# salesforce/ALPRO

Hardware: AMD Instinct MI355X
Metric: video-text pairs/sec (8f x 224^2, 40-tok) (higher is better)
Workload: dtype fp16

## Files before the change

alpro_amd/csrc/attention.hip:

```cpp
#include "common.hpp"
#include "attn_tile.hpp"

namespace alpro {
namespace {

template <typename T> __device__ __forceinline__ int k_swz(int row, int chunk) {
  if (TileCfg<T>::CPR == 8) return chunk ^ ((row >> 1) & 7);
  return chunk ^ (row & 15);
}

template <typename T> struct Col4;
template <> struct Col4<float> {
  typedef u32x4 type;
  static __device__ __forceinline__ u32x4 load(const char* v, int key0, int d) {
    const float* p = (const float*)(v + key0 * TileCfg<float>::RB) + d;
    return mk4(f2u(p[0]), f2u(p[64]), f2u(p[128]), f2u(p[192]));
  }
};
template <typename T16> struct Col4_16 {
  typedef u32x2 type;
  static __device__ __forceinline__ u32x2 load(const char* v, int key0, int d) {
    const uint16_t* p = (const uint16_t*)(v + key0 * (HD * 2)) + d;
    u32x2 r;
    r.x = (uint32_t)p[0] | ((uint32_t)p[64] << 16);
// ... 156 lines not shown
      for (int r = 0; r < 16; ++r) s[kt][r] = 0.f;
      const int krow = kt * 32 + ql;
#pragma unroll
      for (int ks = 0; ks < C::KS; ++ks) {
        const u32x4 a = *(const u32x4*)(Ks + krow * C::RB + (k_swz<T>(krow, 2 * ks + g) << 4));
        mma_chunk<T>(s[kt], a, qf[ks]);
      }
      __builtin_amdgcn_sched_barrier(0);
    }
    const float l_se = softmax_tiles<NKT>(s, scale, [&](int kt, int rq) { return *(const float4*)(Bs + kt * 32 + 8 * rq + 4 * g); });
    if (lse && g == 0 && q < L) lse[((int64_t)b * H + h) * L + q] = l_se;
    if (drop_seed) {
      const uint32_t th = drop_thresh24(drop_p);
      const float ks = 1.0f / (1.0f - drop_p);
      const uint64_t base_i = (((uint64_t)b * H + h) * L + (uint64_t)qc) * L;
#pragma unroll
      for (int kt = 0; kt < NKT; ++kt)
#pragma unroll
        for (int r = 0; r < 16; ++r) s[kt][r] = drop_keep(drop_seed, base_i + kt * 32 + acc_row(r, lane), th) ? s[kt][r] * ks : 0.f;
    }

    f32x16 o[2];
#pragma unroll
    for (int dt = 0; dt < 2; ++dt)
#pragma unroll
      for (int r = 0; r < 16; ++r) o[dt][r] = 0.f;
    pv_tiles<T, NKT>(o, s, Vs, lane);
    if (q < L) store_row64<T>(out + ((int64_t)b * L + q) * H * HD + h * HD, o, lane);
  }
}

__device__ u32x4 g_attn_zero[4];

template <typename T> struct ClsSplit;
template <> struct ClsSplit<f16_t> { static constexpr int NS = 2; static constexpr float C1 = 2048.f, C2 = 1.f; };
template <> struct ClsSplit<bf16_t> { static constexpr int NS = 3; static constexpr float C1 = 1.f, C2 = 1.f; };
template <typename T> __device__ __forceinline__ void cls_split(float x, float& p0, float& p1, float& p2) {
  p0 = quantize<T>(x);
  const float r1 = (x - p0) * ClsSplit<T>::C1;
  p1 = quantize<T>(r1);
  p2 = ClsSplit<T>::NS == 3 ? quantize<T>((r1 - p1) * ClsSplit<T>::C2) : 0.f;
}
template <typename T> struct ClsTrunc;
template <> struct ClsTrunc<f16_t> { static constexpr uint32_t MASK = 0xFFFFE000u; };
template <> struct ClsTrunc<bf16_t> { static constexpr uint32_t MASK = 0xFFFF0000u; };
__device__ __forceinline__ float and_bits(float x, uint32_t m) { return __builtin_bit_cast(float, __builtin_bit_cast(uint32_t, x) & m); }

template <typename T> __device__ __forceinline__ float cls_join(float v0, float v1, float v2) {
  float r = fmaf(v1, 1.0f / ClsSplit<T>::C1, v0);
  if (ClsSplit<T>::NS == 3) r = fmaf(v2, 1.0f / (ClsSplit<T>::C1 * ClsSplit<T>::C2), r);
  return r;
}

template <int N> __device__ __forceinline__ float dpp_from_above(float v) {
  return __builtin_bit_cast(float, __builtin_amdgcn_update_dpp(0, __builtin_bit_cast(int, v), 0x100 + N, 0xf, 0xf, true));
}
template <int N> __device__ __forceinline__ float dpp_from_below(float v) {
  return __builtin_bit_cast(float, __builtin_amdgcn_update_dpp(0, __builtin_bit_cast(int, v), 0x110 + N, 0xf, 0xf, true));
}

template <typename T, int NKT, bool HAS_BIAS, bool CLS = false, bool DROP = false>
__global__ __launch_bounds__(256, 2) void attn_fwd16_kernel(const T* __restrict__ qkv, T* __restrict__ out, int L, int H, float scale,
                                                            const float* __restrict__ key_bias, float* __restrict__ lse, float drop_p,
                                                            uint32_t drop_seed, int order, const float* __restrict__ cls_q, int cls_group,
                                                            float* __restrict__ cls_out) {
  static_assert(sizeof(T) == 2, "16-bit storage only");
  constexpr int LP = NKT * 32, RB = 128;
  constexpr int NS = ClsSplit<T>::NS;
  extern __shared__ __attribute__((aligned(16))) char smem[];
  char* Ks = smem;
  char* Vs = smem + LP * RB;
  char* Os = smem + 2 * LP * RB;
  constexpr bool HALF = NKT == 8;
  constexpr int OW = HALF ? 2048 : 4096;
  float* Bs = (float*)(Os + 4 * OW);
  const int tid = threadIdx.x, lane = tid & 63, wave = __builtin_amdgcn_readfirstlane(tid >> 6);
  int b, h;
  attn_unit(blockIdx.x, gridDim.x, H, order, b, h);
  for (int c = tid; c < LP; c += 256) Bs[c] = c < L ? (HAS_BIAS ? key_bias[(int64_t)b * L + c] * LOG2E : 0.f) : -INFINITY;
  const int64_t ldq = 3 * (int64_t)H * HD;
  const T* base = qkv + (int64_t)b * L * ldq + h * HD;
  const int nqt = (L + 31) >> 5;
  const int g = lane >> 5, ql = lane & 31;

  int cls_tile = -1, c0 = 0, ntile = nqt;
  if (CLS && cls_q) {
    c0 = L - 32 * (nqt - 1);
    if ((c0 & 15) + NS > 16) c0 = (c0 | 15) + 1;
    cls_tile = nqt - 1;
    if (c0 + NS > 32) { c0 = 0; cls_tile = nqt; ntile = nqt + 1; }
  }

// ... 364 lines not shown
                  const float* cls_q, int cls_group, float* cls_out, hipStream_t st) {
  const int nkt = (L + 31) / 32;
  if constexpr (sizeof(T) == 2) {
#define ALPRO_ATTN16(N)                                                                                       \
  return key_bias ? launch_attn16<T, N, true>(qkv, out, batch, L, H, scale, key_bias, lse, dp, ds, cls_q, cls_group, cls_out, st)         \
                  : launch_attn16<T, N, false>(qkv, out, batch, L, H, scale, key_bias, lse, dp, ds, cls_q, cls_group, cls_out, st)
    if (nkt <= 2) ALPRO_ATTN16(2);
    if (nkt <= 4) ALPRO_ATTN16(4);
    if (nkt <= 7) ALPRO_ATTN16(7);
    ALPRO_ATTN16(8);
#undef ALPRO_ATTN16
  }
  if (nkt <= 2) return launch_attn<T, 2>(qkv, out, batch, L, H, scale, key_bias, lse, dp, ds, st);
  if (nkt <= 4) return launch_attn<T, 4>(qkv, out, batch, L, H, scale, key_bias, lse, dp, ds, st);
  if (nkt <= 7) return launch_attn<T, 7>(qkv, out, batch, L, H, scale, key_bias, lse, dp, ds, st);
  return launch_attn<T, 8>(qkv, out, batch, L, H, scale, key_bias, lse, dp, ds, st);
}

}
}

using namespace alpro;

extern "C" int alpro_attn_fwd(const void* qkv, void* out, int dtype, int batch, int L, int H, float scale,
                              const float* key_bias, float* lse, float drop_p, uint32_t drop_seed, const float* cls_q, int cls_group, float* cls_out,
                              void* stream) {
  ALPRO_CHECK(!cls_q || (cls_out && cls_group > 0 && batch % cls_group == 0 && dtype != ALPRO_F32 && ((uintptr_t)cls_q % 16) == 0 && ((uintptr_t)cls_out % 16) == 0),
              "alpro_attn_fwd: the precise CLS query needs cls_out, a group size dividing the batch, 16-byte aligned fp32 side tensors and a 16-bit operand dtype");
  ALPRO_CHECK(qkv && out && batch > 0 && H > 0, "alpro_attn_fwd: bad args");
  ALPRO_CHECK(L > 0 && L <= ALPRO_ATTN_MAX_L, "alpro_attn_fwd: L=%d unsupported (1..%d = ALPRO_ATTN_MAX_L)", L, ALPRO_ATTN_MAX_L);
  ALPRO_CHECK(((uintptr_t)qkv % 16) == 0 && ((uintptr_t)out % 16) == 0, "alpro_attn_fwd: pointers must be 16-byte aligned");
  ALPRO_CHECK(!drop_seed || (drop_p > 0.f && drop_p < 1.f), "alpro_attn_fwd: dropout needs 0 < p < 1");
  if (L > 256) return attn_long_fwd(qkv, out, dtype, batch, L, H, scale, key_bias, lse, drop_p, drop_seed, cls_q, cls_group, cls_out, (hipStream_t)stream);
  ALPRO_DISPATCH_DTYPE(dtype, T, return dispatch_attn<T>(qkv, out, batch, L, H, scale, key_bias, lse, drop_p, drop_seed, cls_q, cls_group, cls_out, (hipStream_t)stream));
  return ALPRO_OK;
}

extern "C" int alpro_attn_temporal_fwd_drop(const void* qkv, void* out, int dtype, int64_t rows, int T, int H, float scale, float* lse, float drop_p,
                                            uint32_t drop_seed, void* stream) {
  ALPRO_CHECK(qkv && out && rows > 0 && H > 0, "alpro_attn_temporal_fwd: bad args");
  ALPRO_CHECK(T > 0 && T <= ALPRO_ATTN_MAX_T, "alpro_attn_temporal_fwd: num_frm=%d unsupported (1..%d = ALPRO_ATTN_MAX_T)", T, ALPRO_ATTN_MAX_T);
  ALPRO_CHECK(rows % T == 0, "alpro_attn_temporal_fwd: rows=%lld not a multiple of T=%d", (long long)rows, T);
  ALPRO_CHECK(((uintptr_t)qkv % 16) == 0 && ((uintptr_t)out % 16) == 0, "alpro_attn_temporal_fwd: pointers must be 16-byte aligned");
  ALPRO_CHECK(drop_p >= 0.f && drop_p < 1.f, "alpro_attn_temporal_fwd: drop_p=%g out of range (dropout needs 0 <= p < 1)", (double)drop_p);
  if (drop_p == 0.f) drop_seed = 0;
  hipStream_t st = (hipStream_t)stream;
  if (32 % T != 0) return attn_temporal_any_fwd(qkv, out, dtype, rows, T, H, scale, lse, drop_p, drop_seed, st);
  const int64_t units = ((rows + 31) / 32) * H;
  int64_t grid = (units + 3) / 4;
  if (grid > 256 * 8) grid = 256 * 8;
  if (dtype != ALPRO_F32) {
    const size_t lds16 = 4 * 3 * 4096;
    static DeviceOnce once_bf16, once_f16, once_bf16_drop, once_f16_drop;
    set_lds_once(once_bf16, attn_temporal_fwd16_kernel<bf16_t>, lds16);
    set_lds_once(once_f16, attn_temporal_fwd16_kernel<f16_t>, lds16);
    set_lds_once(once_bf16_drop, attn_temporal_fwd16_drop_kernel<bf16_t>, lds16);
    set_lds_once(once_f16_drop, attn_temporal_fwd16_drop_kernel<f16_t>, lds16);
    if (grid > 512) grid = 512;
    if (drop_seed) {
      if (dtype == ALPRO_BF16)
        hipLaunchKernelGGL(attn_temporal_fwd16_drop_kernel<bf16_t>, dim3((unsigned)grid), dim3(256), lds16, st, (const bf16_t*)qkv, (bf16_t*)out, rows, T, H, scale, units, lse, drop_p, drop_seed);
      else
        hipLaunchKernelGGL(attn_temporal_fwd16_drop_kernel<f16_t>, dim3((unsigned)grid), dim3(256), lds16, st, (const f16_t*)qkv, (f16_t*)out, rows, T, H, scale, units, lse, drop_p, drop_seed);
    } else if (dtype == ALPRO_BF16)
      hipLaunchKernelGGL(attn_temporal_fwd16_kernel<bf16_t>, dim3((unsigned)grid), dim3(256), lds16, st, (const bf16_t*)qkv, (bf16_t*)out, rows, T, H, scale, units, lse);
    else
// ... 17 lines not shown
```

alpro_amd/csrc/attn_tile.hpp:

```cpp
#pragma once
#include "common.hpp"

namespace alpro {
namespace {

constexpr int HD = 64;
constexpr float LOG2E = 1.4426950408889634f;
constexpr float LN2 = 0.69314718055994531f;

typedef short s16x4 __attribute__((ext_vector_type(4)));

template <typename T> struct TileCfg {
  static constexpr int E = sizeof(T);
  static constexpr int CN = 16 / E;
  static constexpr int RB = HD * E;
  static constexpr int CPR = RB / 16;
  static constexpr int KS = CPR / 2;
  static constexpr int CPT = 16 / CN;
};

template <typename T> __device__ __forceinline__ int u_swz(int row, int chunk) {
  if (TileCfg<T>::CPR == 8) return chunk ^ ((((row >> 1) & 1) << 2) | ((row >> 2) & 3));
  return chunk ^ (row & 15);
}
// ... 8 lines not shown
  const int row = krow0 + (p >> 2);
  const int ch = seg * 2 + ((p >> 1) & 1);
  typedef bf16_t T16;
  return ds_read_tr16(tile + row * TileCfg<T16>::RB + (u_swz<T16>(row, ch) << 4) + ((p & 1) << 3));
}

template <typename T> __device__ __forceinline__ u32x4 load_t_chunk(const char* tile, int row0, int cc, int lane, int dt);
template <> __device__ __forceinline__ u32x4 load_t_chunk<float>(const char* tile, int row0, int cc, int lane, int dt) {
  const int d = dt * 32 + (lane & 31), r = row0 + 8 * cc + 4 * (lane >> 5);
  uint32_t v[4];
#pragma unroll
  for (int e = 0; e < 4; ++e) v[e] = *(const uint32_t*)(tile + tile_off<float>(r + e, d >> 2) + ((d & 3) << 2));
  return mk4(v[0], v[1], v[2], v[3]);
}
template <typename T> __device__ __forceinline__ u32x4 load_t_chunk16(const char* tile, int row0, int cc, int lane, int dt) {
  const int g = lane >> 5;
  const u32x2 a = tr_quad(tile, row0 + 16 * cc + 4 * g, lane, dt);
  const u32x2 b = tr_quad(tile, row0 + 16 * cc + 8 + 4 * g, lane, dt);
  const uint32_t ax = a.x, ay = a.y, bx = b.x, by = b.y;
  return mk4(ax, ay, bx, by);
}
template <> __device__ __forceinline__ u32x4 load_t_chunk<bf16_t>(const char* tile, int row0, int cc, int lane, int dt) { return load_t_chunk16<bf16_t>(tile, row0, cc, lane, dt); }
template <> __device__ __forceinline__ u32x4 load_t_chunk<f16_t>(const char* tile, int row0, int cc, int lane, int dt) { return load_t_chunk16<f16_t>(tile, row0, cc, lane, dt); }

__device__ __forceinline__ uint64_t temporal_drop_base(int64_t r0, int ql, int Tn, int H, int h) {
  const int lg = ql / Tn;
  return (((uint64_t)(r0 / Tn + lg) * H + h) * Tn + (uint64_t)(ql - lg * Tn)) * Tn - (uint64_t)(lg * Tn);
}
__device__ __forceinline__ uint64_t temporal_drop_base_key(int64_t r0, int ql, int Tn, int H, int h) {
  const int lg = ql / Tn;
  return (((uint64_t)(r0 / Tn + lg) * H + h) * Tn - (uint64_t)(lg * Tn)) * Tn + (uint64_t)(ql - lg * Tn);
}

template <typename T> __device__ __forceinline__ void store_quad(T* dst, const float* v) {
  if constexpr (sizeof(T) == 4) {
    *(float4*)dst = make_float4(v[0], v[1], v[2], v[3]);
  } else {
    u32x2 u;
    u.x = pack2(v[0], v[1], (T*)0);
    u.y = pack2(v[2], v[3], (T*)0);
    *(u32x2*)dst = u;
  }
}
template <typename T> __device__ __forceinline__ void store_row64(T* row, const f32x16 (&o)[2], int lane) {
  const int g = lane >> 5;
#pragma unroll
  for (int dt = 0; dt < 2; ++dt)
#pragma unroll
    for (int rq = 0; rq < 4; ++rq) {
      const float v[4] = {o[dt][4 * rq], o[dt][4 * rq + 1], o[dt][4 * rq + 2], o[dt][4 * rq + 3]};
      store_quad<T>(row + dt * 32 + 8 * rq + 4 * g, v);
    }
}

}
}
```

alpro_amd/csrc/common.hpp:

```cpp
#pragma once
#include <hip/hip_runtime.h>
#include <stdint.h>

#include "../../include/alpro_hip.h"

namespace alpro {

typedef float f32x4 __attribute__((ext_vector_type(4)));
typedef uint32_t u32x4 __attribute__((ext_vector_type(4)));
typedef uint32_t u32x2 __attribute__((ext_vector_type(2)));
__device__ __forceinline__ u32x4 mk4(uint32_t a, uint32_t b, uint32_t c, uint32_t d) { return u32x4{a, b, c, d}; }
__device__ __forceinline__ u32x2 mk2(uint32_t a, uint32_t b) { return u32x2{a, b}; }
__device__ __forceinline__ float u2f(uint32_t u) { return __builtin_bit_cast(float, u); }
__device__ __forceinline__ uint32_t f2u(float f) { return __builtin_bit_cast(uint32_t, f); }
typedef float f32x16 __attribute__((ext_vector_type(16)));
typedef __bf16 bf16x8_t __attribute__((ext_vector_type(8)));
typedef _Float16 f16x8_t __attribute__((ext_vector_type(8)));

struct bf16_t { uint16_t v; };
struct f16_t { uint16_t v; };

__device__ __forceinline__ float to_f32(float x) { return x; }
__device__ __forceinline__ float to_f32(bf16_t x) { return __builtin_bit_cast(float, (uint32_t)x.v << 16); }
__device__ __forceinline__ float to_f32(f16_t x) { return (float)__builtin_bit_cast(_Float16, x.v); }
// ... 176 lines not shown
  return DropBase{(uint32_t)base, hi * 0x85EBCA77u, (hi + 1u) * 0x85EBCA77u};
}
__device__ __forceinline__ bool drop_keep(uint32_t seed, const DropBase& b, uint32_t k, uint32_t thresh24) {
  const uint32_t lo = b.lo + k;
  return (mix32(seed ^ (lo * 0x9E3779B1u) ^ (lo < b.lo ? b.h1 : b.h0)) >> 8) >= thresh24;
}
__host__ __device__ inline uint32_t drop_thresh24(float p) { return (uint32_t)(p * 16777216.0f + 0.5f); }

__device__ __forceinline__ void dma16(const void* src, uint32_t lds_addr) {
#pragma clang diagnostic push
#pragma clang diagnostic ignored "-Winline-asm"
  asm volatile("s_mov_b32 m0, %1\n\ts_nop 0\n\tglobal_load_lds_dwordx4 %0, off" ::"v"(src), "s"(lds_addr) : "memory", "m0");
#pragma clang diagnostic pop
}
__device__ __forceinline__ void dma16_sbase(uint32_t voff, const char* sbase, uint32_t lds_addr) {
#pragma clang diagnostic push
#pragma clang diagnostic ignored "-Winline-asm"
  asm volatile("s_mov_b32 m0, %2\n\ts_nop 0\n\tglobal_load_lds_dwordx4 %0, %1" ::"v"(voff), "s"(sbase), "s"(lds_addr) : "memory", "m0");
#pragma clang diagnostic pop
}
__device__ __forceinline__ void store16_sc1(void* p, const u32x4& v) {
  asm volatile("global_store_dwordx4 %0, %1, off sc1\n\ts_nop 1" ::"v"(p), "v"(v) : "memory");
}
__device__ __forceinline__ float sload_f32(const float* p, uint32_t idx) {
  return *((const __attribute__((address_space(4))) float*)p + __builtin_amdgcn_readfirstlane(idx));
}
__device__ __forceinline__ uint32_t lds_addr_of(const void* p) { return (uint32_t)(uintptr_t)(__attribute__((address_space(3))) const char*)p; }

void set_error(const char* fmt, ...);
int attn_long_fwd(const void* qkv, void* out, int dtype, int batch, int L, int H, float scale, const float* key_bias, float* lse, float drop_p,
                  uint32_t drop_seed, const float* cls_q, int cls_group, float* cls_out, hipStream_t st);
int attn_long_bwd(const void* qkv, const void* out, const void* dout, const float* lse, void* dqkv, int dtype, int batch, int L, int H, float scale,
                  const float* key_bias, float drop_p, uint32_t drop_seed, hipStream_t st);
int attn_temporal_any_fwd(const void* qkv, void* out, int dtype, int64_t rows, int T, int H, float scale, float* lse, float drop_p, uint32_t drop_seed,
                          hipStream_t st);
int attn_temporal_any_bwd(const void* qkv, const void* out, const void* dout, const float* lse, void* dqkv, int dtype, int64_t rows, int T, int H,
                          float scale, float drop_p, uint32_t drop_seed, hipStream_t st);

__device__ __forceinline__ void attn_unit(int blk, int nblk, int H, int order, int& b, int& h) {
  const int batch = nblk / H;
  if (order == 1 && (batch & 7) == 0) {
    const int x = blk & 7, i = blk >> 3, j = i / H;
    h = i - j * H;
    b = j * 8 + x;
  } else {
    b = blk / H;
    h = blk - b * H;
  }
}
enum { OPT_GEMM_TILE = 0, OPT_GEMM_GRID = 1, OPT_GEMM_TUNE = 2, OPT_TN_SPLITS = 3, OPT_TN_KIND = 4, OPT_GEMM_TAIL = 5, OPT_ATTN_BWD = 6, OPT_ATTN_ORDER = 7, OPT_GEMM_KIND = 8, OPT_CU_BUDGET = 9, OPT_LN_GRID = 10, OPT_GEMM_SCHED = 11, OPT_GEMM_EPI = 12, OPT_COUNT = 13 };
int get_option(int which);
int get_stream_option(int which, hipStream_t st);

constexpr int SCHED_CLAIM0 = 8, SCHED_MAX_WG = 256, SCHED_BLOCK_U32 = SCHED_CLAIM0 + SCHED_MAX_WG;
struct TileSched {
  uint32_t* blk;
  uint32_t* prev;
  uint32_t magic_ntn;
  uint32_t epi;
};
struct SchedLaunch {
  uint32_t* cur = nullptr;
  uint32_t* prev = nullptr;
  void* slot = nullptr;
  SchedLaunch(hipStream_t st, bool enabled);
  void commit(bool launched);
  ~SchedLaunch();
};
int sched_set_workspace(hipStream_t st, void* ptr, size_t bytes);
inline uint32_t magic_u32(uint32_t d) { return (uint32_t)(((1ull << 32) + d - 1) / d); }
inline int cu_budget(hipStream_t st) {
  int v = get_stream_option(OPT_CU_BUDGET, st);
  if (v < 0) v = get_option(OPT_CU_BUDGET);
  return (v >= 64 && v < 256) ? (v / 8 * 8) : 256;
}

struct DeviceOnce {
  unsigned long long mask = 0;
  template <typename F> void run(F&& f) {
    int dev = 0;
    (void)hipGetDevice(&dev);
    const unsigned long long bit = 1ull << (dev & 63);
    if (!(__atomic_load_n(&mask, __ATOMIC_ACQUIRE) & bit)) {
// ... 27 lines not shown
```

alpro_amd/csrc/runtime.hip:

```cpp
#include <stdarg.h>
#include <stdio.h>
#include <stdlib.h>
#include <string.h>

#include "common.hpp"

namespace alpro {

static thread_local char g_err[512] = "";

void set_error(const char* fmt, ...) {
  va_list ap;
  va_start(ap, fmt);
  vsnprintf(g_err, sizeof(g_err), fmt, ap);
  va_end(ap);
}

namespace {
const char* const kOptNames[OPT_COUNT] = {"gemm_tile", "gemm_grid", "gemm_tune", "tn_splits", "tn_kind", "gemm_tail", "attn_bwd", "attn_order", "gemm_kind", "cu_budget", "ln_grid", "gemm_sched", "gemm_epi"};
const char* const kOptEnv[OPT_COUNT] = {"ALPRO_GEMM_TILE", "ALPRO_GEMM_GRID", "ALPRO_GEMM_TUNE", "ALPRO_TN_SPLITS", "ALPRO_TN_KIND", "ALPRO_GEMM_TAIL", "ALPRO_ATTN_BWD", "ALPRO_ATTN_ORDER", "ALPRO_GEMM_KIND", "ALPRO_CU_BUDGET", "ALPRO_LN_GRID", "ALPRO_GEMM_SCHED", "ALPRO_GEMM_EPI"};
int g_opts[OPT_COUNT];
bool option_allowed(int which, int value) {
  if (which == OPT_GEMM_TUNE) return value >= 0 && value <= 2;
  if (which == OPT_TN_KIND) return value == 0 || value == 2;
  if (which == OPT_ATTN_BWD) return value >= 0 && value <= 2;
  return value >= 0;
}
struct OptInit {
  OptInit() {
    for (int i = 0; i < OPT_COUNT; ++i) {
      const char* e = getenv(kOptEnv[i]);
      const int dflt = (i == OPT_GEMM_TUNE || i == OPT_GEMM_TAIL || i == OPT_ATTN_BWD || i == OPT_GEMM_KIND || i == OPT_GEMM_SCHED || i == OPT_GEMM_EPI) ? 1
                       : i == OPT_TN_KIND ? 2
                                          : 0;
      g_opts[i] = e ? atoi(e) : dflt;
      if (!option_allowed(i, g_opts[i])) {
        fprintf(stderr, "libalpro_hip: %s=%d selected an ablation that has been removed (ignored)\n", kOptEnv[i], g_opts[i]);
        g_opts[i] = dflt;
      }
    }
  }
} g_opt_init;
}

int get_option(int which) { return __atomic_load_n(&g_opts[which], __ATOMIC_RELAXED); }

namespace {
struct StreamOpt { hipStream_t st; int which, value; };
constexpr int kMaxStreamOpts = 32;
StreamOpt g_sopts[kMaxStreamOpts];
int g_nsopts = 0;
int g_sopt_lock = 0;
struct SpinGuard {
  SpinGuard() { while (__atomic_exchange_n(&g_sopt_lock, 1, __ATOMIC_ACQUIRE)) {} }
  ~SpinGuard() { __atomic_store_n(&g_sopt_lock, 0, __ATOMIC_RELEASE); }
};
}

int get_stream_option(int which, hipStream_t st) {
  if (__atomic_load_n(&g_nsopts, __ATOMIC_RELAXED) == 0) return -1;
  SpinGuard g;
  for (int i = 0; i < g_nsopts; ++i)
    if (g_sopts[i].st == st && g_sopts[i].which == which) return g_sopts[i].value;
  return -1;
}
// ... 190 lines not shown
```

alpro_amd/hip.py:

```python
import ctypes
import os

import torch

_HERE = os.path.dirname(os.path.abspath(__file__))
LIB_PATH = os.environ.get("ALPRO_HIP_LIB") or os.path.join(_HERE, "lib", "libalpro_hip.so")

F32, BF16, F16 = 0, 1, 2
ACT_NONE, ACT_GELU, ACT_RELU, ACT_GELU_BWD, ACT_GELU_SAVE_GRAD, ACT_MUL_SAVED, ACT_RELU_MASK = 0, 1, 2, 3, 4, 5, 6
POOL_MODES = {"mean": 0, "max": 1, "lse": 2}
MAP_IDENTITY, MAP_SKIP_CLS, MAP_FRAME_TOKENS, MAP_PATCH_EMBED = 0, 1, 2, 3
ADD_IDENTITY, ADD_PRE_SPATIAL, ADD_PRE_MLP, ADD_PRE_TEMPORAL = 0, 1, 2, 3
EMIT_NONE, EMIT_ROWS, EMIT_FRAME, EMIT_SKIP_CLS = 0, 1, 2, 3
POOL_TEMPORAL, POOL_SPATIAL, POOL_NONE = 0, 1, 2

_TORCH_DTYPE = {F32: torch.float32, BF16: torch.bfloat16, F16: torch.float16}
_CODE = {v: k for k, v in _TORCH_DTYPE.items()}

EXPORTS = ["alpro_hip_last_error", "alpro_hip_abi_version", "alpro_hip_set_option", "alpro_hip_set_stream_option", "alpro_gemm", "alpro_gemm_c2_tiled_rows", "alpro_layernorm_fwd",
           "alpro_attn_temporal_fwd", "alpro_attn_fwd", "alpro_patchify", "alpro_cls_mean_residual",
           "alpro_vit_final_pool", "alpro_bert_embed_fwd", "alpro_cast_from_f32", "alpro_attn_bwd", "alpro_attn_temporal_bwd",
           "alpro_layernorm_bwd", "alpro_transpose", "alpro_transpose_batch", "alpro_gelu_bwd", "alpro_cls_mean_bwd", "alpro_scatter_add_rows", "alpro_gather_cast", "alpro_sumsq", "alpro_adamw_step", "alpro_gemm_tn_acc", "alpro_gemm_tn_acc_ws", "alpro_gemm_tn_workspace_bytes", "alpro_gemm_tn_ranges", "alpro_colsum_acc", "alpro_softmax_xent", "alpro_vtc_loss_fwd", "alpro_vtc_loss_bwd", "alpro_prepare_clips", "alpro_loss_scale_update", "alpro_add_layernorm_fwd", "alpro_layernorm_bwd_emit", "alpro_gemm_batch", "alpro_tproj_small", "alpro_attn_cls_fwd", "alpro_gemm_rows_f32", "alpro_gather_seq_fwd", "alpro_gather_seq_bwd", "alpro_scatter_add_rows_ordered",
           "alpro_hip_sched_workspace_bytes", "alpro_hip_set_sched_workspace", "alpro_hip_release_stream", "alpro_gemm_qkv_tattn", "alpro_add_layernorm_pre_mlp2", "alpro_adamw_step_lp",
           "alpro_gemm_rows_f32_relu_mask", "alpro_clip_pool", "alpro_adamw_step_groups", "alpro_attn_temporal_fwd_drop", "alpro_attn_temporal_bwd_drop",
# ... 94 lines not shown
    lib.alpro_attn_fwd.argtypes = [vp, vp, i32, i32, i32, i32, f32, vp, vp, f32, u32, vp, i32, vp, vp]
    lib.alpro_attn_cls_fwd.argtypes = [vp, i32, vp, vp, vp, i32, i32, i32, i32, f32, f32, u32, vp]
    lib.alpro_gemm_rows_f32.argtypes = [vp, i64, vp, i64, vp, i64, i32, i32, i32, vp, i32, vp, vp, i64, vp, vp, f32, vp]
    lib.alpro_gemm_rows_f32_relu_mask.argtypes = [vp, i64, vp, i64, vp, i64, i32, i32, i32, vp, i64, vp]
    lib.alpro_clip_pool.argtypes = [vp, i64, vp, i64, vp, i32, i32, i32, i32, vp]
    lib.alpro_gemm_c2_tiled_rows.argtypes = [i64, i64, i64, i32]
    lib.alpro_gemm_c2_tiled_rows.restype = i64
    lib.alpro_patchify.argtypes = [vp, vp, i32, i32, i32, i32, i32, vp]
    lib.alpro_cls_mean_residual.argtypes = [vp, i64, vp, vp, i64, i32, i32, i32, vp]
    lib.alpro_vit_final_pool.argtypes = [vp, vp, vp, f32, vp, vp, i32, i32, i32, i32, i32, vp]
    lib.alpro_vit_final_pool_mode.argtypes = [vp, vp, vp, f32, vp, vp, i32, i32, i64, i32, i32, i32, i32, vp]
    lib.alpro_vit_final_pool_mode_bwd.argtypes = [vp, vp, vp, f32, vp, vp, vp, i32, i64, i32, i32, i32, i32, vp, i32, vp, i32, vp, ctypes.c_size_t, vp]
    lib.alpro_add_layernorm_pre_mlp2.argtypes = [vp, vp, vp, vp, i32, vp, vp, vp, f32, vp, i64, i32, i32, i32, vp]
    lib.alpro_bert_embed_fwd.argtypes = [vp, vp, vp, vp, vp, vp, f32, vp, vp, i32, vp, vp, i32, i32, i32, f32, u32, vp]
    lib.alpro_cast_from_f32.argtypes = [vp, vp, i32, i64, vp]
    lib.alpro_hip_set_option.argtypes = [ctypes.c_char_p, i32]
    lib.alpro_hip_set_stream_option.argtypes = [vp, ctypes.c_char_p, i32]
    lib.alpro_hip_sched_workspace_bytes.restype = ctypes.c_size_t
    lib.alpro_hip_set_sched_workspace.argtypes = [vp, vp, ctypes.c_size_t]
    lib.alpro_hip_release_stream.argtypes = [vp]
    lib.alpro_gemm_qkv_tattn.argtypes = [vp, i64, vp, i64, vp, vp, i64, i32, i32, i32, i32, i32, f32, vp, i64, vp, vp]
    lib.alpro_scatter_add_rows_ordered.argtypes = [vp, vp, vp, i32, i32, i64, i64, vp, vp]
    lib.alpro_gather_seq_fwd.argtypes = [vp, vp, vp, vp, vp, vp, i32, i32, i32, i32, i32, vp]
    lib.alpro_gather_seq_bwd.argtypes = [vp, vp, i32, vp, vp, vp, vp, i32, i32, i32, i32, i32, i32, vp]
    lib.alpro_prepare_clips.argtypes = [vp, i32, vp, f32, ctypes.POINTER(f32), ctypes.POINTER(f32), vp, vp, vp, i32, i32, i32, i32, vp]
    lib.alpro_vtc_loss_fwd.argtypes = [vp, vp, vp, vp, vp, i32, i32, i32, i32, vp, vp, vp, vp, vp]
    lib.alpro_vtc_loss_bwd.argtypes = [vp, vp, vp, vp, vp, i32, i32, i32, i32, vp, vp, vp, vp, vp, vp, vp, vp, vp, vp, vp, vp]
    if lib.alpro_hip_abi_version() != ABI_VERSION:
        raise RuntimeError("libalpro_hip.so ABI version mismatch")
    _lib = lib
    return lib


_OPTION_DEFAULTS = {"gemm_tile": 0, "gemm_grid": 0, "gemm_tune": 1, "tn_splits": 0, "tn_kind": 2, "gemm_tail": 1, "attn_bwd": 1, "attn_order": 0, "gemm_kind": 1, "cu_budget": 0, "ln_grid": 0, "gemm_sched": 1, "gemm_epi": 1}
_option_values = {}


def set_option(name, value):
    _check(load().alpro_hip_set_option(name.encode(), int(value)), "alpro_hip_set_option")
    _option_values[name] = int(value)


def set_stream_option(name, value, stream=None):
    h = stream if stream is not None else (_stream() if torch.cuda.is_available() else ctypes.c_void_p(0))
    _check(load().alpro_hip_set_stream_option(h, name.encode(), int(value)), "alpro_hip_set_stream_option")
    return h


def _stream_handle(stream):
    if stream is None:
        return _stream()
    return ctypes.c_void_p(stream.cuda_stream) if isinstance(stream, torch.cuda.Stream) else stream


_sched_ws = {}


def set_sched_workspace(stream=None, tensor=None):
    lib = load()
    h = _stream_handle(stream)
    need = int(lib.alpro_hip_sched_workspace_bytes())
    if tensor is None:
        tensor = torch.empty(need, dtype=torch.uint8, device="cuda")
    if not tensor.is_cuda or tensor.numel() * tensor.element_size() < need or not tensor.is_contiguous():
        raise ValueError("set_sched_workspace: a contiguous CUDA tensor of >= %d bytes" % need)
    _check(lib.alpro_hip_set_sched_workspace(h, ctypes.c_void_p(tensor.data_ptr()), tensor.numel() * tensor.element_size()), "alpro_hip_set_sched_workspace")
    _sched_ws[(tensor.device.index, h.value)] = tensor
# ... 772 lines not shown
```

Before: 435.2.

## Add 16-row query-tile attention forward kernel with 8 waves and online softmax

Adds a new forward attention kernel for 16-bit inputs without key bias or dropout, used by default through a new attn_fwd_kind option. Each block runs 8 waves that loop over 16-row query tiles, prefetching the next Q tile. It splits the keys into two halves with online-softmax rescaling, skips dead key tiles, and overlaps the V loads with the QK^T step. The CLS precise-query split is done in registers with DPP lane shuffles. The aim is better occupancy and less padding waste than the older 32-row kernel for short sequences, at the cost of a second large code path that has to match the old numerics, including the CLS split/join.

```diff
diff --git a/alpro_amd/csrc/attention.hip b/alpro_amd/csrc/attention.hip
--- a/alpro_amd/csrc/attention.hip
+++ b/alpro_amd/csrc/attention.hip
@@ -212,32 +212,6 @@
 
 __device__ u32x4 g_attn_zero[4];
 
-template <typename T> struct ClsSplit;
-template <> struct ClsSplit<f16_t> { static constexpr int NS = 2; static constexpr float C1 = 2048.f, C2 = 1.f; };
-template <> struct ClsSplit<bf16_t> { static constexpr int NS = 3; static constexpr float C1 = 1.f, C2 = 1.f; };
-template <typename T> __device__ __forceinline__ void cls_split(float x, float& p0, float& p1, float& p2) {
-  p0 = quantize<T>(x);
-  const float r1 = (x - p0) * ClsSplit<T>::C1;
-  p1 = quantize<T>(r1);
-  p2 = ClsSplit<T>::NS == 3 ? quantize<T>((r1 - p1) * ClsSplit<T>::C2) : 0.f;
-}
-template <typename T> struct ClsTrunc;
-template <> struct ClsTrunc<f16_t> { static constexpr uint32_t MASK = 0xFFFFE000u; };
-template <> struct ClsTrunc<bf16_t> { static constexpr uint32_t MASK = 0xFFFF0000u; };
-__device__ __forceinline__ float and_bits(float x, uint32_t m) { return __builtin_bit_cast(float, __builtin_bit_cast(uint32_t, x) & m); }
-
-template <typename T> __device__ __forceinline__ float cls_join(float v0, float v1, float v2) {
-  float r = fmaf(v1, 1.0f / ClsSplit<T>::C1, v0);
-  if (ClsSplit<T>::NS == 3) r = fmaf(v2, 1.0f / (ClsSplit<T>::C1 * ClsSplit<T>::C2), r);
-  return r;
-}
-
-template <int N> __device__ __forceinline__ float dpp_from_above(float v) {
-  return __builtin_bit_cast(float, __builtin_amdgcn_update_dpp(0, __builtin_bit_cast(int, v), 0x100 + N, 0xf, 0xf, true));
-}
-template <int N> __device__ __forceinline__ float dpp_from_below(float v) {
-  return __builtin_bit_cast(float, __builtin_amdgcn_update_dpp(0, __builtin_bit_cast(int, v), 0x110 + N, 0xf, 0xf, true));
-}
 
 template <typename T, int NKT, bool HAS_BIAS, bool CLS = false, bool DROP = false>
 __global__ __launch_bounds__(256, 2) void attn_fwd16_kernel(const T* __restrict__ qkv, T* __restrict__ out, int L, int H, float scale,
@@ -668,6 +642,8 @@
   ALPRO_CHECK(((uintptr_t)qkv % 16) == 0 && ((uintptr_t)out % 16) == 0, "alpro_attn_fwd: pointers must be 16-byte aligned");
   ALPRO_CHECK(!drop_seed || (drop_p > 0.f && drop_p < 1.f), "alpro_attn_fwd: dropout needs 0 < p < 1");
   if (L > 256) return attn_long_fwd(qkv, out, dtype, batch, L, H, scale, key_bias, lse, drop_p, drop_seed, cls_q, cls_group, cls_out, (hipStream_t)stream);
+  if (dtype != ALPRO_F32 && !key_bias && !drop_seed && get_option(OPT_ATTN_FWD_KIND) == 1)
+    return attn_fwd_q16(qkv, out, dtype, batch, L, H, scale, lse, cls_q, cls_group, cls_out, (hipStream_t)stream);
   ALPRO_DISPATCH_DTYPE(dtype, T, return dispatch_attn<T>(qkv, out, batch, L, H, scale, key_bias, lse, drop_p, drop_seed, cls_q, cls_group, cls_out, (hipStream_t)stream));
   return ALPRO_OK;
 }
diff --git a/alpro_amd/csrc/attention_fwd_q16.hip b/alpro_amd/csrc/attention_fwd_q16.hip
--- /dev/null
+++ b/alpro_amd/csrc/attention_fwd_q16.hip
@@ -0,0 +1,342 @@
+#include "common.hpp"
+#include "attn_tile.hpp"
+#include "gemm_pipe.hpp"
+
+namespace alpro {
+namespace {
+
+__device__ u32x4 g_q16_zero[4];
+
+constexpr int Q16_WAVES = 8, Q16_OW = 2048;
+
+__device__ __forceinline__ int v16_swz(int row) { return (((row >> 1) & 1) << 2) | (((row >> 2) & 1) << 1); }
+__device__ __forceinline__ u32x2 tr_quad_v16(const char* vs, int key0, int lane, int dt) {
+  const int p = lane & 15, row = key0 + (p >> 2);
+  return ds_read_tr16(vs + row * 128 + (((2 * dt) ^ v16_swz(row)) << 4) + ((p & 3) << 3));
+}
+__device__ __forceinline__ float bit_select(uint32_t mask, float a, float b) {
+  return __builtin_bit_cast(float, (__builtin_bit_cast(uint32_t, a) & mask) | (__builtin_bit_cast(uint32_t, b) & ~mask));
+}
+template <int V> struct HalfTag { static constexpr int value = V; };
+
+template <typename T, int NKT, bool CLS>
+__global__ __launch_bounds__(512, 4) void attn_fwd_q16_kernel(const T* __restrict__ qkv, T* __restrict__ out, int L, int H, float scale, float* __restrict__ lse,
+                                                              int order, const float* __restrict__ cls_q, int cls_group, float* __restrict__ cls_out) {
+  static_assert(sizeof(T) == 2, "16-bit storage only");
+  constexpr int LP = NKT * 32, RB = 128;
+  constexpr int NH0 = (NKT + 1) / 2, NH1 = NKT - NH0;
+  constexpr int NS = ClsSplit<T>::NS;
+  constexpr int LMIN = NKT == 2 ? 1 : (NKT == 4 ? 65 : (NKT == 7 ? 129 : 225));
+  extern __shared__ __attribute__((aligned(16))) char smem[];
+  char* Ks = smem;
+  char* Vs = smem + LP * RB;
+  char* Os = smem + 2 * LP * RB;
+  const int tid = threadIdx.x, lane = tid & 63, wave = __builtin_amdgcn_readfirstlane(tid >> 6);
+  int b, h;
+  attn_unit(blockIdx.x, gridDim.x, H, order, b, h);
+  const int64_t ldq = 3 * (int64_t)H * HD;
+  const T* base = qkv + (int64_t)b * L * ldq + h * HD;
+  const int n16 = (L + 15) >> 4;
+  const int g = lane >> 4, ql = lane & 15;
+
+  int cls_tile = -1, c0 = 0, ntile = n16;
+  if (CLS) {
+    c0 = L - 16 * (n16 - 1);
+    cls_tile = n16 - 1;
+    if (c0 + NS > 16) { c0 = 0; cls_tile = n16; ntile = n16 + 1; }
+  }
+
+  constexpr int NP = 4 * NKT, NPW = (NP + Q16_WAVES - 1) / Q16_WAVES;
+  const uint32_t k_lds = lds_addr_of(Ks), v_lds = lds_addr_of(Vs);
+  const char* zero = (const char*)g_q16_zero;
+#pragma unroll
+  for (int i = 0; i < NPW; ++i) {
+    const int piece = wave + Q16_WAVES * i;
+    if (piece < NP) {
+      const int row = piece * 8 + (lane >> 3), slot = lane & 7;
+      const T* src = base + (int64_t)row * ldq;
+      dma16(row < L ? (const char*)(src + H * HD + ((slot ^ ((row >> 1) & 7)) << 3)) : zero, __builtin_amdgcn_readfirstlane(k_lds + piece * 1024));
+    }
+  }
+  auto load_q = [&](int qt, u32x4(&qf)[2]) __attribute__((always_inline)) {
+    const int qc = min(qt * 16 + ql, L - 1);
+#pragma unroll
+    for (int ks = 0; ks < 2; ++ks) qf[ks] = *(const u32x4*)(base + (int64_t)qc * ldq + (g + 4 * ks) * 8);
+    if constexpr (CLS) {
+      if (qt == cls_tile) {
+        const float* cq = cls_q + (int64_t)(b / cls_group) * ldq + h * HD;
+        const int j = ql - c0;
+#pragma unroll
+        for (int ks = 0; ks < 2; ++ks) {
+          const float4 a = *(const float4*)(cq + (g + 4 * ks) * 8), c = *(const float4*)(cq + (g + 4 * ks) * 8 + 4);
+          const float x[8] = {a.x, a.y, a.z, a.w, c.x, c.y, c.z, c.w};
+          float part[8];
+#pragma unroll
+          for (int e = 0; e < 8; ++e) {
+            const float p0 = and_bits(x[e], ClsTrunc<T>::MASK);
+            const float r1 = (x[e] - p0) * ClsSplit<T>::C1;
+            float p1 = r1, p2 = 0.f;
+            if (NS == 3) { p1 = and_bits(r1, ClsTrunc<T>::MASK); p2 = (r1 - p1) * ClsSplit<T>::C2; }
+            part[e] = j == 0 ? p0 : (j == 1 ? p1 : p2);
+          }
+          const u32x4 pk = pack_chunk<T>(part);
+          if (j >= 0 && j < NS) qf[ks] = pk;
+        }
+      }
+    }
+  };
+  int seq = (wave + (int)(blockIdx.x >> 3)) & 7;
+  int swap_a = -1, swap_b = -1;
+  if (CLS && cls_tile == ntile - 1 && cls_tile >= 8 && ntile < 16) { swap_a = cls_tile; swap_b = 7; }
+  auto tile_at = [&](int pos) __attribute__((always_inline)) { return pos == swap_a ? swap_b : (pos == swap_b ? swap_a : pos); };
+  bool has = seq < ntile;
+  int qt = tile_at(has ? seq : 0);
+  u32x4 qf[2], qn[2];
+  load_q(qt, qf);
+  int nv = 0;
+#pragma unroll
+  for (int i = 0; i < NPW; ++i) {
+    const int piece = wave + Q16_WAVES * i;
+    if (piece < NP) {
+      const int row = piece * 8 + (lane >> 3), slot = lane & 7;
+      const T* src = base + (int64_t)row * ldq;
+      dma16(row < L ? (const char*)(src + 2 * H * HD + ((slot ^ v16_swz(row)) << 3)) : zero, __builtin_amdgcn_readfirstlane(v_lds + piece * 1024));
+      ++nv;
+    }
+  }
+  if (nv == NPW) wait_vmcnt<NPW>();
+  else wait_vmcnt<NPW - 1>();
+  __syncthreads();
+
+  const float sl = scale * LOG2E;
+  char* Ow = Os + wave * Q16_OW;
+  bool v_pending = true;
+  f32x4 s[2 * NH0];
+  f32x4 o[4];
+  float m = 0.f, lsum = 0.f;
+
+  auto half = [&](auto tag) __attribute__((always_inline)) {
+    constexpr int HV = decltype(tag)::value;
+    constexpr int KT0 = HV == 0 ? 0 : 2 * NH0, NT = 2 * (HV == 0 ? NH0 : NH1);
+    const bool cls_here = CLS && qt == cls_tile;
+    auto live = [&](int t) __attribute__((always_inline)) { return (KT0 + t + 1) * 16 <= LMIN || KT0 + t < n16; };
+    auto partial = [&](int t) __attribute__((always_inline)) { return (KT0 + t + 1) * 16 > LMIN && (KT0 + t + 1) * 16 > L; };
+#pragma unroll
+    for (int t = 0; t < NT; ++t) {
+      f32x4 acc = {0.f, 0.f, 0.f, 0.f};
+      if (live(t)) {
+        const int krow = (KT0 + t) * 16 + ql;
+#pragma unroll
+        for (int ks = 0; ks < 2; ++ks) {
+          const u32x4 a = *(const u32x4*)(Ks + krow * RB + (((g + 4 * ks) ^ ((krow >> 1) & 7)) << 4));
+          acc = Mma16<T>::run(a, qf[ks], acc);
+        }
+      }
+      s[t] = acc;
+      if (t & 1) __builtin_amdgcn_sched_barrier(0);
+    }
+    if constexpr (HV == 0) {
+      const int nseq = seq + Q16_WAVES;
+      if (nseq < ntile) load_q(tile_at(nseq), qn);
+    }
+    if constexpr (CLS) {
+      if (cls_here) {
+        int qo = ql;
+        asm volatile("" : "+v"(qo));
+        const float w1 = qo == c0 ? 1.0f / ClsSplit<T>::C1 : 0.f, w2 = qo == c0 ? 1.0f / (ClsSplit<T>::C1 * ClsSplit<T>::C2) : 0.f;
+        const uint32_t sel1 = qo == c0 + 1 ? 0xFFFFFFFFu : 0u, sel2 = (NS == 3 && qo == c0 + 2) ? 0xFFFFFFFFu : 0u;
+#pragma unroll
+        for (int t = 0; t < NT; ++t)
+#pragma unroll
+          for (int r = 0; r < 4; ++r) {
+            const float a = s[t][r];
+            float v = fmaf(dpp_from_above<1>(a), w1, a);
+            if (NS == 3) v = fmaf(dpp_from_above<2>(a), w2, v);
+            float w = bit_select(sel1, dpp_from_below<1>(v), v);
+            if (NS == 3) w = bit_select(sel2, dpp_from_below<2>(v), w);
+            s[t][r] = w;
+          }
+      }
+    }
+    float mx = -INFINITY;
+    int lim = L - 4 * g;
+    asm volatile("" : "+v"(lim));
+#pragma unroll
+    for (int t = 0; t < NT; ++t) {
+      if (live(t)) {
+        if (partial(t)) {
+#pragma unroll
+          for (int r = 0; r < 4; ++r) s[t][r] = (KT0 + t) * 16 + r < lim ? s[t][r] : -INFINITY;
+        }
+        mx = fmaxf(fmaxf(mx, fmaxf(s[t][0], s[t][1])), fmaxf(s[t][2], s[t][3]));
+      }
+    }
+    mx = fmaxf(mx, __shfl_xor(mx, 16, 64));
+    mx = fmaxf(mx, __shfl_xor(mx, 32, 64));
+    mx *= sl;
+    if constexpr (HV == 0) {
+      m = mx;
+    } else {
+      const float mn = fmaxf(m, mx);
+      const float alpha = __builtin_amdgcn_exp2f(m - mn);
+      m = mn;
+      lsum *= alpha;
+#pragma unroll
+      for (int dt = 0; dt < 4; ++dt)
+#pragma unroll
+        for (int r = 0; r < 4; ++r) o[dt][r] *= alpha;
+    }
+    const float nm = -m;
+#pragma unroll
+    for (int t = 0; t < NT; ++t) {
+      if (live(t)) {
+#pragma unroll
+        for (int r = 0; r < 4; ++r) {
+          const float pr = __builtin_amdgcn_exp2f(fmaf(s[t][r], sl, nm));
+          s[t][r] = pr;
+          lsum += pr;
+        }
+      }
+    }
+    if constexpr (CLS) {
+      if (cls_here) {
+        int qo = ql;
+        asm volatile("" : "+v"(qo));
+        const uint32_t part = (qo >= c0 && qo < c0 + NS) ? 0xFFFFFFFFu : 0u;
+        const uint32_t tm = part ? ClsTrunc<T>::MASK : 0xFFFFFFFFu;
+        const uint32_t sel1 = qo == c0 + 1 ? 0xFFFFFFFFu : 0u, sel2 = (NS == 3 && qo == c0 + 2) ? 0xFFFFFFFFu : 0u;
+#pragma unroll
+        for (int t = 0; t < NT; ++t)
+#pragma unroll
+          for (int r = 0; r < 4; ++r) {
+            const float pr = s[t][r];
+            const float h0 = and_bits(pr, tm);
+            const float r1 = (pr - h0) * ClsSplit<T>::C1;
+            float w;
+            if (NS == 2) {
+              w = bit_select(sel1, r1, h0);
+            } else {
+              const float h1 = and_bits(r1, ClsTrunc<T>::MASK);
+              const float r2 = (r1 - h1) * ClsSplit<T>::C2;
+              w = bit_select(sel1, h1, h0);
+              w = bit_select(sel2, r2, w);
+            }
+            s[t][r] = w;
+          }
+      }
+    }
+    if (v_pending) {
+      wait_vmcnt<0>();
+      __syncthreads();
+      v_pending = false;
+    }
+#pragma unroll
+    for (int u = 0; u < NT / 2; ++u) {
+      if (live(2 * u)) {
+        const float pv[8] = {s[2 * u][0], s[2 * u][1], s[2 * u][2], s[2 * u][3], s[2 * u + 1][0], s[2 * u + 1][1], s[2 * u + 1][2], s[2 * u + 1][3]};
+        const u32x4 pb = pack_chunk<T>(pv);
+        const int key0 = (KT0 + 2 * u) * 16 + 4 * g;
+#pragma unroll
+        for (int dt = 0; dt < 4; ++dt) {
+          const u32x2 lo = tr_quad_v16(Vs, key0, lane, dt), hi = tr_quad_v16(Vs, key0 + 16, lane, dt);
+          const uint32_t a0 = lo.x, a1 = lo.y, a2 = hi.x, a3 = hi.y;
+          o[dt] = Mma16<T>::run(mk4(a0, a1, a2, a3), pb, o[dt]);
+        }
+      }
+      __builtin_amdgcn_sched_barrier(0);
+    }
+  };
+
+  while (has) {
+#pragma unroll
+    for (int dt = 0; dt < 4; ++dt) o[dt] = f32x4{0.f, 0.f, 0.f, 0.f};
+    lsum = 0.f;
+#pragma unroll
+    for (int ks = 0; ks < 2; ++ks) qn[ks] = qf[ks];
+    half(HalfTag<0>{});
+    if (NH0 * 32 < LMIN || NH0 * 32 < L) half(HalfTag<1>{});
+    lsum += __shfl_xor(lsum, 16, 64);
+    lsum += __shfl_xor(lsum, 32, 64);
+    const float inv = 1.0f / lsum;
+    int le = lane;
+    asm volatile("" : "+v"(le));
+    const int ge = le >> 4, qe = le & 15;
+    const int q = qt * 16 + qe;
+    if (lse && ge == 0 && q < L) lse[((int64_t)b * H + h) * L + q] = (m + __builtin_amdgcn_logf(lsum)) * LN2;
+    if constexpr (CLS) {
+      if (qt == cls_tile) {
+        float* dst = cls_out + (int64_t)b * H * HD + h * HD;
+#pragma unroll
+        for (int dt = 0; dt < 4; ++dt) {
+          float v[4];
+#pragma unroll
+          for (int e = 0; e < 4; ++e) {
+            const float a = o[dt][e];
+            const float b1 = dpp_from_above<1>(a), b2 = NS == 3 ? dpp_from_above<2>(a) : 0.f;
+            v[e] = cls_join<T>(a, b1, b2) * inv;
+          }
+          if (qe == c0) *(float4*)(dst + dt * 16 + 4 * ge) = make_float4(v[0], v[1], v[2], v[3]);
+        }
+      }
+    }
+#pragma unroll
+    for (int dt = 0; dt < 4; ++dt) {
+      const uint32_t lo = pack2(o[dt][0] * inv, o[dt][1] * inv, (T*)0);
+      const uint32_t hi = pack2(o[dt][2] * inv, o[dt][3] * inv, (T*)0);
+      *(u32x2*)(Ow + qe * 128 + (((dt * 2 + (ge >> 1)) ^ ((qe >> 1) & 7)) << 4) + (ge & 1) * 8) = mk2(lo, hi);
+    }
+    wait_lgkmcnt0();
+#pragma unroll
+    for (int p = 0; p < 2; ++p) {
+      const int row = p * 8 + (le >> 3), slot = le & 7;
+      const u32x4 v = *(const u32x4*)(Ow + row * 128 + ((slot ^ ((row >> 1) & 7)) << 4));
+      const int qq = qt * 16 + row;
+      if (qq < L) store16_sc1(out + ((int64_t)b * L + qq) * H * HD + h * HD + slot * 8, v);
+    }
+    asm volatile("" ::: "memory");
+    seq += Q16_WAVES;
+    has = seq < ntile;
+    qt = tile_at(has ? seq : 0);
+#pragma unroll
+    for (int ks = 0; ks < 2; ++ks) qf[ks] = qn[ks];
+  }
+  if (v_pending) {
+    wait_vmcnt<0>();
+    __syncthreads();
+  }
+}
+
+template <typename T, int NKT>
+int launch_q16(const void* qkv, void* out, int batch, int L, int H, float scale, float* lse, const float* cls_q, int cls_group, float* cls_out, hipStream_t st) {
+  const size_t lds = 2 * (size_t)NKT * 32 * 128 + (size_t)Q16_WAVES * Q16_OW;
+  static DeviceOnce once_plain, once_cls;
+  set_lds_once(once_plain, attn_fwd_q16_kernel<T, NKT, false>, lds);
+  set_lds_once(once_cls, attn_fwd_q16_kernel<T, NKT, true>, lds);
+  const int order = get_option(OPT_ATTN_ORDER);
+  if (cls_q)
+    hipLaunchKernelGGL((attn_fwd_q16_kernel<T, NKT, true>), dim3(batch * H), dim3(64 * Q16_WAVES), lds, st, (const T*)qkv, (T*)out, L, H, scale, lse, order, cls_q, cls_group, cls_out);
+  else
+    hipLaunchKernelGGL((attn_fwd_q16_kernel<T, NKT, false>), dim3(batch * H), dim3(64 * Q16_WAVES), lds, st, (const T*)qkv, (T*)out, L, H, scale, lse, order, cls_q, cls_group, cls_out);
+  return check_launch("alpro_attn_fwd");
+}
+
+template <typename T>
+int dispatch_q16(const void* qkv, void* out, int batch, int L, int H, float scale, float* lse, const float* cls_q, int cls_group, float* cls_out, hipStream_t st) {
+  const int nkt = (L + 31) / 32;
+  if (nkt <= 2) return launch_q16<T, 2>(qkv, out, batch, L, H, scale, lse, cls_q, cls_group, cls_out, st);
+  if (nkt <= 4) return launch_q16<T, 4>(qkv, out, batch, L, H, scale, lse, cls_q, cls_group, cls_out, st);
+  if (nkt <= 7) return launch_q16<T, 7>(qkv, out, batch, L, H, scale, lse, cls_q, cls_group, cls_out, st);
+  return launch_q16<T, 8>(qkv, out, batch, L, H, scale, lse, cls_q, cls_group, cls_out, st);
+}
+
+}
+
+int attn_fwd_q16(const void* qkv, void* out, int dtype, int batch, int L, int H, float scale, float* lse, const float* cls_q, int cls_group, float* cls_out,
+                 hipStream_t st) {
+  if (dtype == ALPRO_BF16) return dispatch_q16<bf16_t>(qkv, out, batch, L, H, scale, lse, cls_q, cls_group, cls_out, st);
+  if (dtype == ALPRO_F16) return dispatch_q16<f16_t>(qkv, out, batch, L, H, scale, lse, cls_q, cls_group, cls_out, st);
+  set_error("attn_fwd_q16: 16-bit operand dtypes only (got %d)", dtype);
+  return ALPRO_ERR_INVALID;
+}
+
+}
diff --git a/alpro_amd/csrc/attn_tile.hpp b/alpro_amd/csrc/attn_tile.hpp
--- a/alpro_amd/csrc/attn_tile.hpp
+++ b/alpro_amd/csrc/attn_tile.hpp
@@ -64,6 +64,36 @@
   return (((uint64_t)(r0 / Tn + lg) * H + h) * Tn - (uint64_t)(lg * Tn)) * Tn + (uint64_t)(ql - lg * Tn);
 }
 
+template <typename T> struct ClsSplit;
+template <> struct ClsSplit<f16_t> { static constexpr int NS = 2; static constexpr float C1 = 2048.f, C2 = 1.f; };
+template <> struct ClsSplit<bf16_t> { static constexpr int NS = 3; static constexpr float C1 = 1.f, C2 = 1.f; };
+template <typename T> __device__ __forceinline__ void cls_split(float x, float& p0, float& p1, float& p2) {
+  p0 = quantize<T>(x);
+  const float r1 = (x - p0) * ClsSplit<T>::C1;
+  p1 = quantize<T>(r1);
+  p2 = ClsSplit<T>::NS == 3 ? quantize<T>((r1 - p1) * ClsSplit<T>::C2) : 0.f;
+}
+template <typename T> struct ClsTrunc;
+template <> struct ClsTrunc<f16_t> { static constexpr uint32_t MASK = 0xFFFFE000u; };
+template <> struct ClsTrunc<bf16_t> { static constexpr uint32_t MASK = 0xFFFF0000u; };
+__device__ __forceinline__ float and_bits(float x, uint32_t m) { return __builtin_bit_cast(float, __builtin_bit_cast(uint32_t, x) & m); }
+
+template <typename T> __device__ __forceinline__ float cls_join(float v0, float v1, float v2) {
+  float r = fmaf(v1, 1.0f / ClsSplit<T>::C1, v0);
+  if (ClsSplit<T>::NS == 3) r = fmaf(v2, 1.0f / (ClsSplit<T>::C1 * ClsSplit<T>::C2), r);
+  return r;
+}
+
+template <int N> __device__ __forceinline__ float dpp_from_above(float v) {
+  return __builtin_bit_cast(float, __builtin_amdgcn_update_dpp(0, __builtin_bit_cast(int, v), 0x100 + N, 0xf, 0xf, true));
+}
+template <int N> __device__ __forceinline__ float dpp_from_below(float v) {
+  return __builtin_bit_cast(float, __builtin_amdgcn_update_dpp(0, __builtin_bit_cast(int, v), 0x110 + N, 0xf, 0xf, true));
+}
+
+template <int N> __device__ __forceinline__ void wait_vmcnt() { asm volatile("s_waitcnt vmcnt(%0)" ::"n"(N) : "memory"); }
+__device__ __forceinline__ void wait_lgkmcnt0() { asm volatile("s_waitcnt lgkmcnt(0)" ::: "memory"); }
+
 template <typename T> __device__ __forceinline__ void store_quad(T* dst, const float* v) {
   if constexpr (sizeof(T) == 4) {
     *(float4*)dst = make_float4(v[0], v[1], v[2], v[3]);
diff --git a/alpro_amd/csrc/common.hpp b/alpro_amd/csrc/common.hpp
--- a/alpro_amd/csrc/common.hpp
+++ b/alpro_amd/csrc/common.hpp
@@ -232,6 +232,8 @@
                   uint32_t drop_seed, const float* cls_q, int cls_group, float* cls_out, hipStream_t st);
 int attn_long_bwd(const void* qkv, const void* out, const void* dout, const float* lse, void* dqkv, int dtype, int batch, int L, int H, float scale,
                   const float* key_bias, float drop_p, uint32_t drop_seed, hipStream_t st);
+int attn_fwd_q16(const void* qkv, void* out, int dtype, int batch, int L, int H, float scale, float* lse, const float* cls_q, int cls_group, float* cls_out,
+                 hipStream_t st);
 int attn_temporal_any_fwd(const void* qkv, void* out, int dtype, int64_t rows, int T, int H, float scale, float* lse, float drop_p, uint32_t drop_seed,
                           hipStream_t st);
 int attn_temporal_any_bwd(const void* qkv, const void* out, const void* dout, const float* lse, void* dqkv, int dtype, int64_t rows, int T, int H,
@@ -248,7 +250,7 @@
     h = blk - b * H;
   }
 }
-enum { OPT_GEMM_TILE = 0, OPT_GEMM_GRID = 1, OPT_GEMM_TUNE = 2, OPT_TN_SPLITS = 3, OPT_TN_KIND = 4, OPT_GEMM_TAIL = 5, OPT_ATTN_BWD = 6, OPT_ATTN_ORDER = 7, OPT_GEMM_KIND = 8, OPT_CU_BUDGET = 9, OPT_LN_GRID = 10, OPT_GEMM_SCHED = 11, OPT_GEMM_EPI = 12, OPT_COUNT = 13 };
+enum { OPT_GEMM_TILE = 0, OPT_GEMM_GRID = 1, OPT_GEMM_TUNE = 2, OPT_TN_SPLITS = 3, OPT_TN_KIND = 4, OPT_GEMM_TAIL = 5, OPT_ATTN_BWD = 6, OPT_ATTN_ORDER = 7, OPT_GEMM_KIND = 8, OPT_CU_BUDGET = 9, OPT_LN_GRID = 10, OPT_GEMM_SCHED = 11, OPT_GEMM_EPI = 12, OPT_ATTN_FWD_KIND = 13, OPT_COUNT = 14 };
 int get_option(int which);
 int get_stream_option(int which, hipStream_t st);
 
diff --git a/alpro_amd/csrc/runtime.hip b/alpro_amd/csrc/runtime.hip
--- a/alpro_amd/csrc/runtime.hip
+++ b/alpro_amd/csrc/runtime.hip
@@ -17,8 +17,8 @@
 }
 
 namespace {
-const char* const kOptNames[OPT_COUNT] = {"gemm_tile", "gemm_grid", "gemm_tune", "tn_splits", "tn_kind", "gemm_tail", "attn_bwd", "attn_order", "gemm_kind", "cu_budget", "ln_grid", "gemm_sched", "gemm_epi"};
-const char* const kOptEnv[OPT_COUNT] = {"ALPRO_GEMM_TILE", "ALPRO_GEMM_GRID", "ALPRO_GEMM_TUNE", "ALPRO_TN_SPLITS", "ALPRO_TN_KIND", "ALPRO_GEMM_TAIL", "ALPRO_ATTN_BWD", "ALPRO_ATTN_ORDER", "ALPRO_GEMM_KIND", "ALPRO_CU_BUDGET", "ALPRO_LN_GRID", "ALPRO_GEMM_SCHED", "ALPRO_GEMM_EPI"};
+const char* const kOptNames[OPT_COUNT] = {"gemm_tile", "gemm_grid", "gemm_tune", "tn_splits", "tn_kind", "gemm_tail", "attn_bwd", "attn_order", "gemm_kind", "cu_budget", "ln_grid", "gemm_sched", "gemm_epi", "attn_fwd_kind"};
+const char* const kOptEnv[OPT_COUNT] = {"ALPRO_GEMM_TILE", "ALPRO_GEMM_GRID", "ALPRO_GEMM_TUNE", "ALPRO_TN_SPLITS", "ALPRO_TN_KIND", "ALPRO_GEMM_TAIL", "ALPRO_ATTN_BWD", "ALPRO_ATTN_ORDER", "ALPRO_GEMM_KIND", "ALPRO_CU_BUDGET", "ALPRO_LN_GRID", "ALPRO_GEMM_SCHED", "ALPRO_GEMM_EPI", "ALPRO_ATTN_FWD_KIND"};
 int g_opts[OPT_COUNT];
 bool option_allowed(int which, int value) {
   if (which == OPT_GEMM_TUNE) return value >= 0 && value <= 2;
@@ -30,7 +30,7 @@
   OptInit() {
     for (int i = 0; i < OPT_COUNT; ++i) {
       const char* e = getenv(kOptEnv[i]);
-      const int dflt = (i == OPT_GEMM_TUNE || i == OPT_GEMM_TAIL || i == OPT_ATTN_BWD || i == OPT_GEMM_KIND || i == OPT_GEMM_SCHED || i == OPT_GEMM_EPI) ? 1
+      const int dflt = (i == OPT_GEMM_TUNE || i == OPT_GEMM_TAIL || i == OPT_ATTN_BWD || i == OPT_GEMM_KIND || i == OPT_GEMM_SCHED || i == OPT_GEMM_EPI || i == OPT_ATTN_FWD_KIND) ? 1
                        : i == OPT_TN_KIND ? 2
                                           : 0;
       g_opts[i] = e ? atoi(e) : dflt;
diff --git a/alpro_amd/hip.py b/alpro_amd/hip.py
--- a/alpro_amd/hip.py
+++ b/alpro_amd/hip.py
@@ -150,7 +150,7 @@
     return lib
 
 
-_OPTION_DEFAULTS = {"gemm_tile": 0, "gemm_grid": 0, "gemm_tune": 1, "tn_splits": 0, "tn_kind": 2, "gemm_tail": 1, "attn_bwd": 1, "attn_order": 0, "gemm_kind": 1, "cu_budget": 0, "ln_grid": 0, "gemm_sched": 1, "gemm_epi": 1}
+_OPTION_DEFAULTS = {"gemm_tile": 0, "gemm_grid": 0, "gemm_tune": 1, "tn_splits": 0, "tn_kind": 2, "gemm_tail": 1, "attn_bwd": 1, "attn_order": 0, "gemm_kind": 1, "cu_budget": 0, "ln_grid": 0, "gemm_sched": 1, "gemm_epi": 1, "attn_fwd_kind": 1}
 _option_values = {}
 
 
```

Result: no change. 434.6 (median of 2 runs) (-0.1%).
